# hank-kuo-cs/Volumetric-Primitives-Net

Hardware: NVIDIA B200
Metric: primitive-loss fwd+bwd samples/sec (higher is better)
Workload: dtype f32

## Files before the change

### volumetric-primitives-net_b200/csrc/chamfer_prep.cu

```cuda
#include "common.cuh"

namespace vpn {

constexpr int kSortThreads = 1024;
constexpr int kSortMaxM = 16384;
constexpr int kBlk = 128;

__device__ __forceinline__ float prep_inf() { return __int_as_float(0x7f800000); }
__device__ __forceinline__ unsigned spread6(unsigned x) {
  x = (x | (x << 8)) & 0x0000300Fu;
  x = (x | (x << 4)) & 0x000030C3u;
  x = (x | (x << 2)) & 0x00009249u;
  return x;
}
__device__ __forceinline__ u64 prep_pk(float a, float b) { u64 r; asm("mov.b64 %0, {%1,%2};" : "=l"(r) : "f"(a), "f"(b)); return r; }
__device__ __forceinline__ void prep_upk(u64 v, float& a, float& b) { asm("mov.b64 {%0,%1}, %2;" : "=f"(a), "=f"(b) : "l"(v)); }
__device__ __forceinline__ u64 prep_sub2(u64 a, u64 b) { u64 r; asm("sub.rn.f32x2 %0, %1, %2;" : "=l"(r) : "l"(a), "l"(b)); return r; }
__device__ __forceinline__ u64 prep_mul2(u64 a, u64 b) { u64 r; asm("mul.rn.f32x2 %0, %1, %2;" : "=l"(r) : "l"(a), "l"(b)); return r; }
__device__ __forceinline__ u64 prep_fma2(u64 a, u64 b, u64 c) { u64 r; asm("fma.rn.f32x2 %0, %1, %2, %3;" : "=l"(r) : "l"(a), "l"(b), "l"(c)); return r; }

__device__ __forceinline__ float warp_min_f(float v) { float r; asm volatile("redux.sync.min.f32 %0, %1, 0xffffffff;" : "=f"(r) : "f"(v)); return r; }
__device__ __forceinline__ float warp_max_f(float v) { float r; asm volatile("redux.sync.max.f32 %0, %1, 0xffffffff;" : "=f"(r) : "f"(v)); return r; }

__device__ __forceinline__ void prep_block_box(float (&lo)[3], float (&hi)[3], unsigned amu, float (*red)[7]) {
// ... 318 lines not shown
    __syncthreads();
    pp.mark();
    return;
  }
  const int b = blockIdx.x;
  const float* T = p2 + (size_t)b * M * 3;
  float* Ts = p2s + (size_t)b * M * 3;
  float4* Tv = p2v + (size_t)b * nchunks * kBlk;
  int* pm = perm + (size_t)b * M;
  float* cb = cbox + (size_t)b * nchunks * 8;
  if (M <= 8 * kSortThreads) prep_sort_targets<8>(T, Ts, Tv, pm, cb, tmax + b, M, sort_targets, deterministic, nchunks, cnt, start, ent, wsum, red, pp);
  else prep_sort_targets<16>(T, Ts, Tv, pm, cb, tmax + b, M, sort_targets, deterministic, nchunks, cnt, start, ent, wsum, red, pp);
}

constexpr int kNearRows = 8, kRepsRows = 4;
constexpr int kNearCols = 32, kRepsCols = 4;
constexpr int kMaxNear = 32, kMaxReps = 128;
constexpr int kGapCap = 1024;
constexpr int kBoundWarps = 4;

__device__ __forceinline__ float box_gap2(const float* __restrict__ a, const float* __restrict__ b) {
  float s = 0.f;
#pragma unroll
  for (int k = 0; k < 3; ++k) {
    const float g = fmaxf(0.f, fmaxf(a[k] - b[3 + k], b[k] - a[3 + k]));
    s = fmaf(g, g, s);
  }
  return s;
}

__global__ void __launch_bounds__(kBoundWarps * 32, 8)
chamfer_prune_bounds_kernel(const float* __restrict__ p1, const float* __restrict__ p2s,
                            const float* __restrict__ rbox, const float* __restrict__ cbox,
                            float* __restrict__ rthr, float* __restrict__ cub, int P, int M, int nrb, int nchunks,
                            int near_rows, int reps_rows, int near_cols, int reps_cols, int gap_cap) {
  extern __shared__ unsigned s_gap[];
  __shared__ float4 s_reps[kBoundWarps][2 * kMaxReps];
  __shared__ int s_sel[kBoundWarps][kMaxNear];
  const int b = blockIdx.y, lane = threadIdx.x & 31, warp = threadIdx.x >> 5;
  const int id = blockIdx.x * kBoundWarps + warp;
  if (id >= nrb + nchunks) return;
  unsigned* gap = s_gap + warp * gap_cap; float4* reps = s_reps[warp]; int* sel = s_sel[warp];
  const bool is_row = id >= nchunks;
  const int blk = is_row ? id - nchunks : id;
  const int n_mine = is_row ? P : M, n_other = is_row ? M : P;
  const float* mine = (is_row ? p1 + (size_t)b * P * 3 : p2s + (size_t)b * M * 3);
  const float* other = (is_row ? p2s + (size_t)b * M * 3 : p1 + (size_t)b * P * 3);
  const int nob = is_row ? nchunks : nrb;
  const float* obox = (is_row ? cbox + (size_t)b * nchunks * 8 : rbox + (size_t)b * nrb * 8);
  const int near = is_row ? near_rows : near_cols, per = is_row ? reps_rows : reps_cols;
  const float* mb = is_row ? rbox + ((size_t)b * nrb + blk) * 8 : cbox + ((size_t)b * nchunks + blk) * 8;
  float mybox[6];
#pragma unroll
  for (int k = 0; k < 6; ++k) mybox[k] = mb[k];
  float x[4], y[4], z[4]; bool valid[4];
#pragma unroll
  for (int u = 0; u < 4; ++u) {
    const int idx = blk * kBlk + u * 32 + lane;
    valid[u] = idx < n_mine;
    x[u] = y[u] = z[u] = 0.f;
    if (valid[u]) { x[u] = mine[3 * (size_t)idx]; y[u] = mine[3 * (size_t)idx + 1]; z[u] = mine[3 * (size_t)idx + 2]; }
  }
  const int stride = (nob + kGapCap - 1) / kGapCap, ncand = (nob + stride - 1) / stride;
  unsigned lmin = 0xffffffffu;
  for (int c = lane; c < ncand; c += 32) {
    const float4* ob = reinterpret_cast<const float4*>(obox + (size_t)c * stride * 8);
    const float4 o0 = ob[0], o1 = ob[1];
    const float other_box[6] = {o0.x, o0.y, o0.z, o0.w, o1.x, o1.y};
    const float g = box_gap2(mybox, other_box);
    const unsigned k = ((g == g) ? (__float_as_uint(g) & ~0x3ffu) : 0x7f800000u) | (unsigned)c;
    gap[c] = k;
    lmin = min(lmin, k);
  }
  const int nsel = min(near, ncand);
  for (int s = 0; s < nsel; ++s) {
    const unsigned w = __reduce_min_sync(0xffffffffu, lmin);
    const int bi = (w == 0xffffffffu) ? -1 : (int)(w & 0x3ffu);
    if (lane == 0) sel[s] = bi < 0 ? 0 : bi;
    if (bi >= 0 && (bi & 31) == lane) {
      gap[bi] = 0xffffffffu;
      lmin = 0xffffffffu;
      for (int c = lane; c < ncand; c += 32) lmin = min(lmin, gap[c]);
    }
  }
  __syncwarp();
  const int nrep = nsel * per;
  for (int i = lane; i < nrep; i += 32) {
    const int ob = sel[i / per] * stride;
    int o = ob * kBlk + (i % per) * (kBlk / per);
    o = min(o, n_other - 1);
    const float qx = other[3 * (size_t)o], qy = other[3 * (size_t)o + 1], qz = other[3 * (size_t)o + 2];
    reps[2 * i] = make_float4(qx, qx, qy, qy); reps[2 * i + 1] = make_float4(qz, qz, 0.f, 0.f);
  }
  __syncwarp();
  const u64 x01 = prep_pk(x[0], x[1]), x23 = prep_pk(x[2], x[3]), y01 = prep_pk(y[0], y[1]), y23 = prep_pk(y[2], y[3]),
            z01 = prep_pk(z[0], z[1]), z23 = prep_pk(z[2], z[3]);
  float ub[4] = {prep_inf(), prep_inf(), prep_inf(), prep_inf()};
  for (int r = 0; r < nrep; ++r) {
    const ulonglong2 qa = *reinterpret_cast<const ulonglong2*>(&reps[2 * r]);
    const u64 qz = *reinterpret_cast<const u64*>(&reps[2 * r + 1]);
    const u64 dx0 = prep_sub2(x01, qa.x), dy0 = prep_sub2(y01, qa.y), dz0 = prep_sub2(z01, qz);
    const u64 dx1 = prep_sub2(x23, qa.x), dy1 = prep_sub2(y23, qa.y), dz1 = prep_sub2(z23, qz);
    const u64 s0 = prep_fma2(dz0, dz0, prep_fma2(dy0, dy0, prep_mul2(dx0, dx0)));
    const u64 s1 = prep_fma2(dz1, dz1, prep_fma2(dy1, dy1, prep_mul2(dx1, dx1)));
    float a, c, e, f;
    prep_upk(s0, a, c); prep_upk(s1, e, f);
    ub[0] = fminf(ub[0], a); ub[1] = fminf(ub[1], c); ub[2] = fminf(ub[2], e); ub[3] = fminf(ub[3], f);
  }
  float m = 0.f;
#pragma unroll
  for (int u = 0; u < 4; ++u) if (valid[u]) m = fmaxf(m, ub[u]);
  m = warp_max_f(m);
  if (lane == 0) { if (is_row) rthr[(size_t)b * nrb + blk] = m; else cub[(size_t)b * nchunks + blk] = m; }
}

int chamfer_row_segment() { return kRowSeg; }

size_t chamfer_sort_smem_bytes(int M) {
  if (M > kSortMaxM) return 0;
  return (size_t)kCells * 8 + (((size_t)M * 4 + 15) & ~(size_t)15);
}

int chamfer_prep_launch(const float* p1, const float* p2, float* p2s, float4* p2v, int* perm, float* cbox, float* rbox, float* rthr,
                        float* cub, float* tmax, float* p1s, int* rperm, unsigned long long* stats, int B, int P, int M, cudaStream_t s) {
  const int nchunks = (M + kBlk - 1) / kBlk, nrb = (P + kBlk - 1) / kBlk;
  const size_t smem_t = chamfer_sort_smem_bytes(M);
  const size_t smem_r = (size_t)kCells * 8 + (size_t)kRowSeg * 4 + (size_t)kRowSeg * 12;
  const size_t smem = smem_t > smem_r ? smem_t : smem_r;
  static DeviceOnce once;
  if (set_dyn_smem(chamfer_sort_targets_kernel, kCells * 8 + kSortMaxM * 4 + kRowSeg * 12, once) != cudaSuccess) {
    vpn_set_error("chamfer prep: smem attribute"); return VPN_ERR_CUDA;
  }
  const long long seg_ctas = (long long)((P + kRowSeg - 1) / kRowSeg) * B;
  if (B + seg_ctas > 0x7fffffffLL) { vpn_set_error("chamfer prep: too many row segments"); return VPN_ERR_SHAPE; }
  chamfer_sort_targets_kernel<<<(unsigned)(B + seg_ctas), kSortThreads, smem, s>>>(p2, p2s, p2v, perm, cbox, tmax, M, smem_t > 0 ? 1 : 0, nchunks,
                                                                                   p1, p1s, rperm, rbox, P, nrb, B,
                                                                                   tuning_value(kTunePrepDeterministic) == 1 ? 1 : 0,
                                                                                   tuning_value(kTunePrepProbe) == 1 ? stats : nullptr);
  int rc = vpn_check_launch("chamfer_sort_targets_kernel");
  if (rc) return rc;
  auto pick = [](int key, int dflt, int cap) { const int v = tuning_value(key); return (v >= 1 && v <= cap && (key == kTunePrepNearRows || key == kTunePrepNearCols || v == 1 || v == 2 || v == 4)) ? v : dflt; };
  const int most = nrb > nchunks ? nrb : nchunks;
  const int gap_cap = most >= kGapCap ? kGapCap : ((most + 31) & ~31);
  chamfer_prune_bounds_kernel<<<dim3((nrb + nchunks + kBoundWarps - 1) / kBoundWarps, B), kBoundWarps * 32,
                                (size_t)kBoundWarps * gap_cap * sizeof(unsigned), s>>>(
      p1s, p2s, rbox, cbox, rthr, cub, P, M, nrb, nchunks, pick(kTunePrepNearRows, kNearRows, kMaxNear), pick(kTunePrepRepsRows, kRepsRows, 4),
      pick(kTunePrepNearCols, kNearCols, kMaxNear), pick(kTunePrepRepsCols, kRepsCols, 4), gap_cap);
  return vpn_check_launch("chamfer_prune_bounds_kernel");
}

}
```

### volumetric-primitives-net_b200/csrc/chamfer_tc.cu

```cuda
#include <cuda_fp16.h>
#include "common.cuh"

namespace vpn {

constexpr int kTcBlk = 128;
constexpr int kTcEpiWarps = 16;
constexpr int kTcThreads = (kTcEpiWarps + 4) * 32;
constexpr int kTcBlkBytes = kTcBlk * 32;
constexpr float kTcBig = 1.0e30f;
constexpr int kTcDefaultHunits = 0;

__device__ __forceinline__ uint32_t tc_smem_u32(const void* p) { return (uint32_t)__cvta_generic_to_shared(p); }
__device__ __forceinline__ float tc_inf() { return __int_as_float(0x7f800000); }

__device__ __forceinline__ uint64_t tc_desc(uint32_t saddr) {
  return (uint64_t)((saddr & 0x3FFFF) >> 4) | ((uint64_t)(128 >> 4) << 16) | ((uint64_t)(256 >> 4) << 32) | (1ull << 46);
}
constexpr uint32_t kTcIdesc = (1u << 4) | (0u << 7) | (0u << 10) | ((uint32_t)(2 * kTcBlk >> 3) << 17) | ((uint32_t)(kTcBlk >> 4) << 24);

constexpr uint32_t kTcIdescHalf = (1u << 4) | (0u << 7) | (0u << 10) | ((uint32_t)(kTcBlk >> 3) << 17) | ((uint32_t)(kTcBlk >> 4) << 24);
constexpr uint32_t kTcIdescHalfF16 = (0u << 4) | (0u << 7) | (0u << 10) | ((uint32_t)(kTcBlk >> 3) << 17) | ((uint32_t)(kTcBlk >> 4) << 24);

__device__ __forceinline__ void tc_mma(uint32_t d_tmem, uint64_t a, uint64_t b, uint32_t accumulate, uint32_t idesc = kTcIdesc) {
#if defined(VPN_TC_VARIANT) && VPN_TC_VARIANT == 3
// ... 181 lines not shown
  uint32_t u23 = tc_min_s16x2(__byte_perm(m2, m3, 0x5410), __byte_perm(m2, m3, 0x7632));
  u01 = tc_max_s16x2(u01, 0u); u23 = tc_max_s16x2(u23, 0u);
  const float2 f01 = __half22float2(*reinterpret_cast<const __half2*>(&u01)), f23 = __half22float2(*reinterpret_cast<const __half2*>(&u23));
  u[0] = f01.x; u[1] = f01.y; u[2] = f23.x; u[3] = f23.y;
  return fminf(tc_min3(u[0], u[1], u[2]), u[3]);
}

__device__ __forceinline__ u64 tc_spread_nibbles(uint32_t v) {
  u64 x = v;
  x = (x | (x << 16)) & 0x0000FFFF0000FFFFull;
  x = (x | (x << 8)) & 0x00FF00FF00FF00FFull;
  x = (x | (x << 4)) & 0x0F0F0F0F0F0F0F0Full;
  return x;
}
__device__ __forceinline__ float tc_box_gap2(const float* __restrict__ a, const float* __restrict__ b) {
  float s = 0.f;
#pragma unroll
  for (int k = 0; k < 3; ++k) {
    const float g = fmaxf(0.f, fmaxf(a[k] - b[3 + k], b[k] - a[3 + k]));
    s = fmaf(g, g, s);
  }
  return s;
}

__device__ __forceinline__ bool tc_pass_needed(int j, int nc, int NB, const uint32_t* raw) {
  const uint32_t live = ~raw[2 * j] | ((2 * j + 1 < nc) ? ~raw[2 * j + 1] : 0u);
  return (live & ((1u << NB) - 1u)) != 0u;
}

constexpr int kPlanThreads = 128;
static_assert(kPlanThreads == kTcPlanWords, "one plan word per thread");
__global__ void __launch_bounds__(kPlanThreads)
chamfer_tc_plan_kernel(const float* __restrict__ cbox, const float* __restrict__ rbox, const float* __restrict__ rthr,
                       const float* __restrict__ cub, uint32_t* __restrict__ plan_masks, int* __restrict__ plan_work,
                       int ncta, int ntiles, int nsplit, int nrb_total, int NB, int nchunks, int cps) {
  __shared__ uint32_t skipR[64], skipC[64];
  __shared__ int s_live[kPlanThreads / 32];
  __shared__ float4 s_rbox[16][2];
  __shared__ float s_rthr[16];
  const int tid = threadIdx.x, lane = tid & 31, warp = tid >> 5;
  const int cta = blockIdx.x;
  const int tile_i = cta % ntiles, split = (cta / ntiles) % nsplit, b = cta / (ntiles * nsplit);
  const int c_first = split * cps, nc = min(nchunks, c_first + cps) - c_first;
  if (tid < 64) { skipR[tid] = 0u; skipC[tid] = 0u; }
  if (tid < 2 * NB) {
    const int r = tid >> 1, rb = tile_i * NB + r;
    if (rb < nrb_total) s_rbox[r][tid & 1] = reinterpret_cast<const float4*>(rbox + ((size_t)b * nrb_total + rb) * 8)[tid & 1];
  } else if (tid >= 32 && tid < 32 + NB) {
    const int r = tid - 32, rb = tile_i * NB + r;
    s_rthr[r] = (rb < nrb_total) ? __fmul_ru(rthr[(size_t)b * nrb_total + rb], 1.00001f) : 0.f;
  }
  __syncthreads();
  {
    const int c = tid & 63, r0 = (tid >> 6) * (NB / 2);
    if (c < nc) {
      const float4 c0 = reinterpret_cast<const float4*>(cbox + ((size_t)b * nchunks + c_first + c) * 8)[0];
      const float4 c1 = reinterpret_cast<const float4*>(cbox + ((size_t)b * nchunks + c_first + c) * 8)[1];
      const float cb8[8] = {c0.x, c0.y, c0.z, c0.w, c1.x, c1.y, c1.z, c1.w};
      const float ub = __fmul_ru(cub[(size_t)b * nchunks + c_first + c], 1.00001f);
      uint32_t mr = 0u, mc = 0u;
      for (int r = r0; r < r0 + NB / 2; ++r) {
        bool pr = true, pc = true;
        if (tile_i * NB + r < nrb_total) {
          const float4 a0 = s_rbox[r][0], a1 = s_rbox[r][1];
          const float rb8[8] = {a0.x, a0.y, a0.z, a0.w, a1.x, a1.y, a1.z, a1.w};
          const float gap2 = tc_box_gap2(rb8, cb8);
          pr = gap2 > s_rthr[r];
          pc = gap2 > ub;
        }
        mr |= pr ? (1u << r) : 0u;
        mc |= pc ? (1u << r) : 0u;
      }
      atomicOr(&skipR[c], mr);
      atomicOr(&skipC[c], mc);
    }
  }
  __syncthreads();
  uint32_t* out = plan_masks + (size_t)cta * kTcPlanWords;
  int live = 0;
  {
    const int c = tid & 63;
    const uint32_t m = (c < nc) ? (tid < 64 ? skipR[c] : skipC[c]) : 0xffffffffu;
    if (c < nc) live = NB - __popc(m & ((1u << NB) - 1u));
    out[tid] = m;
  }
#pragma unroll
  for (int o = 16; o > 0; o >>= 1) live += __shfl_xor_sync(0xffffffffu, live, o);
  if (lane == 0) s_live[warp] = live;
  __syncthreads();
  if (tid == 0) plan_work[cta] = s_live[0] + s_live[1] + s_live[2] + s_live[3];
}

constexpr int kOrderThreads = 1024, kOrderBins = 2112;
__global__ void __launch_bounds__(kOrderThreads)
chamfer_tc_order_kernel(const int* __restrict__ plan_work, int* __restrict__ plan_order, int ncta) {
  __shared__ int hist[kOrderBins];
  const int tid = threadIdx.x;
  for (int i = tid; i < kOrderBins; i += kOrderThreads) hist[i] = 0;
  __syncthreads();
  for (int i = tid; i < ncta; i += kOrderThreads) atomicAdd(&hist[min(max(plan_work[i], 0), kOrderBins - 1)], 1);
  __syncthreads();
  {
    constexpr int kPer = (kOrderBins + kOrderThreads - 1) / kOrderThreads;
    __shared__ int wsum[32];
    const int lane = tid & 31, warp = tid >> 5;
    int cnt[kPer], sum = 0;
#pragma unroll
    for (int k = 0; k < kPer; ++k) { const int w = kOrderBins - 1 - (tid * kPer + k); cnt[k] = (w >= 0) ? hist[w] : 0; sum += cnt[k]; }
    int inc = sum;
#pragma unroll
    for (int o = 1; o < 32; o <<= 1) { const int t = __shfl_up_sync(0xffffffffu, inc, o); if (lane >= o) inc += t; }
    if (lane == 31) wsum[warp] = inc;
    __syncthreads();
    if (warp == 0) {
      const int w = wsum[lane];
// ... 363 lines not shown
          else if (v < bv || j == 0) { bv = v; bj = j; }
        }
      }
      mn[i] = bv; ix[i] = bj;
    }
  }
}

__global__ void __launch_bounds__(256)
chamfer_tc_bounds_kernel(const float* __restrict__ p2, float* __restrict__ tmax, int M) {
  __shared__ float red[8];
  const float* T = p2 + (size_t)blockIdx.x * M * 3;
  float m = 0.f;
  for (int i = threadIdx.x; i < 3 * M; i += 256) {
    const float v = fabsf(T[i]);
    m = (v <= m) ? m : v;
  }
#pragma unroll
  for (int o = 16; o > 0; o >>= 1) { const float x = __shfl_xor_sync(0xffffffffu, m, o); m = (x <= m) ? m : x; }
  if ((threadIdx.x & 31) == 0) red[threadIdx.x >> 5] = m;
  __syncthreads();
  if (threadIdx.x == 0) {
    for (int w = 1; w < 8; ++w) m = (red[w] <= m) ? m : red[w];
    tmax[blockIdx.x] = m;
  }
}

size_t chamfer_tc_smem_bytes(int NB) { return tc_smem_bytes(NB); }
int chamfer_tc_plan_words() { return kTcPlanWords; }


int chamfer_tc_launch(const float* p1, const float* p2, float* rbest, u64* rmask, float* cbest, u64* cmask,
                      float2* tslack, int* fallback, float* tmax, const float* cbox, const float* rbox, const float* rthr,
                      const float* cub, u64* stats, uint32_t* plan_masks, int* plan_work, int* plan_order, int with_bounds,
                      int B, int P, int M, int NB, int ntiles, int nsplit, int nchunks, int cps, cudaStream_t s) {
  static DeviceOnce once;
  const size_t smem = tc_smem_bytes(NB);
  {
    cudaError_t e = set_dyn_smem(chamfer_tc_kernel<0>, (int)tc_smem_bytes(16), once);
    for (int k = 0; k < 4 && e == cudaSuccess; ++k) {
      void (*kern)(const float*, const float*, float*, u64*, float*, u64*, float2*, int*, const float*, const uint32_t*, const int*, u64*,
                   int, int, int, int, int, int, int) = k == 0 ? chamfer_tc_kernel<1> : (k == 1 ? chamfer_tc_kernel<2> : (k == 2 ? chamfer_tc_kernel<3> : chamfer_tc_kernel<4>));
      static DeviceOnce more[4];
      e = set_dyn_smem(kern, (int)tc_smem_bytes(16), more[k]);
    }
    if (e != cudaSuccess) { vpn_set_error("chamfer tc: smem attribute: %s", cudaGetErrorString(e)); return VPN_ERR_CUDA; }
  }
  int rc;
  if (with_bounds) {
    chamfer_tc_bounds_kernel<<<B, 256, 0, s>>>(p2, tmax, M);
    if ((rc = vpn_check_launch("chamfer_tc_bounds_kernel"))) return rc;
  }
  const long long ncta_ll = (long long)ntiles * nsplit * B;
  if (ncta_ll > 0x7fffffffLL) { vpn_set_error("chamfer tc: too many tiles"); return VPN_ERR_SHAPE; }
  const int ncta = (int)ncta_ll;
  if (cbox != nullptr) {
    chamfer_tc_plan_kernel<<<ncta, kPlanThreads, 0, s>>>(
        cbox, rbox, rthr, cub, plan_masks, plan_work, ncta, ntiles, nsplit, (P + kTcBlk - 1) / kTcBlk, NB, nchunks, cps);
    if ((rc = vpn_check_launch("chamfer_tc_plan_kernel"))) return rc;
    chamfer_tc_order_kernel<<<1, kOrderThreads, 0, s>>>(plan_work, plan_order, ncta);
    if ((rc = vpn_check_launch("chamfer_tc_order_kernel"))) return rc;
  }
  const int tune_h = tuning_value(kTuneTcHunits);
  const int hunits = (tune_h >= 1 && tune_h <= 5) ? tune_h - 1 : kTcDefaultHunits;
#define VPN_TC_LAUNCH(H) chamfer_tc_kernel<H><<<ncta, kTcThreads, smem, s>>>(p1, p2, rbest, rmask, cbest, cmask, tslack, fallback, tmax, \
                                                   cbox ? plan_masks : nullptr, cbox ? plan_order : nullptr, stats, \
                                                   ntiles, nsplit, P, M, NB, nchunks, cps)
  switch (hunits) {
    case 0: VPN_TC_LAUNCH(0); break;
    case 1: VPN_TC_LAUNCH(1); break;
    case 2: VPN_TC_LAUNCH(2); break;
    case 3: VPN_TC_LAUNCH(3); break;
    default: VPN_TC_LAUNCH(4); break;
  }
#undef VPN_TC_LAUNCH
  return vpn_check_launch("chamfer_tc_kernel");
}

int chamfer_flagged_launch(const float* p1, const float* p2, float* min1, int* idx1, float* min2, int* idx2,
                           const int* fallback, int B, int P, int M, cudaStream_t s) {
  chamfer_flagged_kernel<<<dim3(32, B), 256, 0, s>>>(p1, p2, min1, idx1, min2, idx2, fallback, P, M);
  return vpn_check_launch("chamfer_flagged_kernel");
}

}
```

### volumetric-primitives-net_b200/csrc/chamfer_tiled.cu

```cuda
#include <cstdlib>
#include <mutex>
#include <type_traits>
#include "common.cuh"

namespace vpn {

enum { MODE_EXACT = 0, MODE_DIFF = 1, MODE_EXPAND = 2, MODE_TC = 3 };

constexpr int kTThreads = 256;
constexpr int kTWarps = kTThreads / 32;
constexpr int kCW = 128;
constexpr int kMaxChunksPerSplit = 64;
constexpr float kBig = 1.0e30f;

__device__ __forceinline__ u64 pk(float a, float b) { u64 r; asm("mov.b64 %0, {%1,%2};" : "=l"(r) : "f"(a), "f"(b)); return r; }
__device__ __forceinline__ void upk(u64 v, float& a, float& b) { asm("mov.b64 {%0,%1}, %2;" : "=f"(a), "=f"(b) : "l"(v)); }
__device__ __forceinline__ u64 add2(u64 a, u64 b) { u64 r; asm("add.rn.f32x2 %0, %1, %2;" : "=l"(r) : "l"(a), "l"(b)); return r; }
__device__ __forceinline__ u64 sub2(u64 a, u64 b) { u64 r; asm("sub.rn.f32x2 %0, %1, %2;" : "=l"(r) : "l"(a), "l"(b)); return r; }
__device__ __forceinline__ u64 mul2(u64 a, u64 b) { u64 r; asm("mul.rn.f32x2 %0, %1, %2;" : "=l"(r) : "l"(a), "l"(b)); return r; }
__device__ __forceinline__ u64 fma2(u64 a, u64 b, u64 c) { u64 r; asm("fma.rn.f32x2 %0, %1, %2, %3;" : "=l"(r) : "l"(a), "l"(b), "l"(c)); return r; }
__device__ __forceinline__ float min3f(float a, float b, float c) { float r; asm("min.f32 %0, %1, %2, %3;" : "=f"(r) : "f"(a), "f"(b), "f"(c)); return r; }
__device__ __forceinline__ float warp_min_f32(float a) { float r; asm volatile("redux.sync.min.f32 %0, %1, 0xffffffff;" : "=f"(r) : "f"(a)); return r; }
__device__ __forceinline__ float inf_f() { return __int_as_float(0x7f800000); }

// ... 559 lines not shown
          }
          int at;
          const int st = unit_scan(d, dm, lane, &at);
          u64 kv = ~0ull;
          if (st == 1) kv = ((u64)__float_as_uint(sqrtf(dm)) << 32) | (unsigned)__float_as_int(rows[base_row + at].w);
          else if (st == 2) kv = unit_exact_walk(tx, ty, tz, rows + base_row, 0, 1);
          best = kv < best ? kv : best;
        }
        if (best != ~0ull) atomicMin(&key2[(size_t)b * M + col], best);
      }
      __syncthreads();
    }
  }
}

__global__ void chamfer_unpack_key_kernel(const u64* __restrict__ key, float* __restrict__ mn, int* __restrict__ idx, size_t n,
                                          const int* __restrict__ skip, int per_sample, const int* __restrict__ perm) {
  size_t i = (size_t)blockIdx.x * blockDim.x + threadIdx.x;
  if (i >= n) return;
  const size_t smp = i / (size_t)per_sample;
  if (skip && skip[smp]) return;
  u64 k = key[i];
  const size_t o = perm ? smp * (size_t)per_sample + (size_t)perm[i] : i;
  mn[o] = __uint_as_float((unsigned)(k >> 32));
  idx[o] = (int)(unsigned)(k & 0xffffffffu);
}

struct TiledPlan { int R, ntiles, nchunks, nsplit, cps, tc, TM; };

size_t chamfer_tc_smem_bytes(int NB);
int chamfer_tc_plan_words();
int chamfer_tc_launch(const float* p1, const float* p2, float* rbest, u64* rmask, float* cbest, u64* cmask,
                      float2* tslack, int* fallback, float* tmax, const float* cbox, const float* rbox, const float* rthr,
                      const float* cub, u64* stats, unsigned* plan_masks, int* plan_work, int* plan_order, int with_bounds,
                      int B, int P, int M, int NB, int ntiles, int nsplit, int nchunks, int cps, cudaStream_t s);
int chamfer_prep_launch(const float* p1, const float* p2, float* p2s, float4* p2v, int* perm, float* cbox, float* rbox, float* rthr,
                        float* cub, float* tmax, float* p1s, int* rperm, unsigned long long* stats, int B, int P, int M, cudaStream_t s);
int chamfer_flagged_launch(const float* p1, const float* p2, float* min1, int* idx1, float* min2, int* idx2,
                           const int* fallback, int B, int P, int M, cudaStream_t s);

static void finish_plan(TiledPlan& pl, int B, long long slots, int min_cps) {
  long long base = (long long)pl.ntiles * B;
  long long s = (4 * slots + base - 1) / base;
  long long smin = (pl.nchunks + kMaxChunksPerSplit - 1) / kMaxChunksPerSplit;
  long long smax = pl.nchunks / min_cps;
  if (s > smax) s = smax;
  if (s < smin) s = smin;
  if (s > pl.nchunks) s = pl.nchunks;
  if (s < 1) s = 1;
  pl.cps = (int)((pl.nchunks + s - 1) / s);
  pl.nsplit = (pl.nchunks + pl.cps - 1) / pl.cps;
}

static bool make_plan(int B, int P, int M, int sm_count, TiledPlan& pl) {
  if (P < 1024 || M < kCW || B < 1) return false;
  pl.tc = 0;
  pl.nchunks = (M + kCW - 1) / kCW;
  const int rs[3] = {16, 8, 4};
  int pick = 4;
  for (int k = 0; k < 3; ++k) {
    int R = rs[k], tm = kTThreads * R;
    long long nt = (P + tm - 1) / tm;
    double waste = (double)(nt * tm) / P;
    long long slots = (long long)sm_count * (R <= 8 ? 2 : 1);
    if (waste <= 1.26 && nt * B * pl.nchunks >= 2 * slots) { pick = R; break; }
  }
  { int r = tuning_value(kTuneTiledR); if (r == 4 || r == 8 || r == 16) pick = r; }
  pl.R = pick;
  pl.TM = kTThreads * pl.R;
  pl.ntiles = (P + pl.TM - 1) / pl.TM;
  finish_plan(pl, B, (long long)sm_count * (pl.R <= 8 ? 2 : 1), 1);
  return pl.nsplit <= 65535;
}

static bool make_plan_tc(int B, int P, int M, int sm_count, TiledPlan& pl) {
  if (P < 512 || M < kCW || B < 1) return false;
  pl.tc = 1;
  pl.nchunks = (M + kCW - 1) / kCW;
  const int nbs[3] = {16, 8, 4};
  int pick = 4;
  for (int k = 0; k < 3; ++k) {
    int nb = nbs[k], tm = 128 * nb;
    long long nt = (P + tm - 1) / tm;
    double waste = (double)(nt * tm) / P;
    if (waste <= 1.26 && nt * B * pl.nchunks >= 2LL * sm_count * 8) { pick = nb; break; }
  }
  { int r = tuning_value(kTuneTcNb); if (r == 4 || r == 8 || r == 16) pick = r; }
  pl.R = pick;
  pl.TM = 128 * pl.R;
  pl.ntiles = (P + pl.TM - 1) / pl.TM;
  finish_plan(pl, B, sm_count, 4);
  return pl.nsplit <= 65535;
}

static size_t al256(size_t x) { return (x + 255) & ~(size_t)255; }

struct TiledWs { size_t rbest, rmask, cbest, cmask, tslack, fallback, tmax, cthr, key2, p2s, p2v, perm, cbox, rbox, rthr, cub, pmask, pwork, porder, p1s, rperm, total; };
static TiledWs ws_layout(int B, int P, int M, const TiledPlan& pl) {
  TiledWs w; size_t o = 0;
  w.rbest = o; o += al256((size_t)B * pl.nsplit * P * 4);
  w.rmask = o; o += al256((size_t)B * pl.nsplit * P * 8 * (pl.tc ? 4 : 1));
  w.cbest = o; o += al256((size_t)B * pl.ntiles * M * 4);
  w.cmask = o; o += al256((size_t)B * pl.ntiles * M * (pl.tc ? 8 : 4));
  w.tslack = o; o += al256((size_t)B * pl.ntiles * 8);
  w.fallback = o; o += al256((size_t)B * 4 + 8 + 128);
  w.tmax = o; o += al256((size_t)B * 4);
  w.cthr = o; o += al256((size_t)B * M * 4);
  w.key2 = o; o += al256((size_t)B * M * 8);
  w.p2s = w.p2v = w.perm = w.cbox = w.rbox = w.rthr = w.cub = w.pmask = w.pwork = w.porder = w.p1s = w.rperm = 0;
  if (pl.tc) {
    const size_t nrb = (size_t)(P + 127) / 128;
    w.p2s = o; o += al256((size_t)B * M * 12);
    w.p2v = o; o += al256((size_t)B * pl.nchunks * kCW * 16);
    w.perm = o; o += al256((size_t)B * M * 4);
    w.cbox = o; o += al256((size_t)B * pl.nchunks * 32);
    w.rbox = o; o += al256((size_t)B * nrb * 32);
    w.rthr = o; o += al256((size_t)B * nrb * 4);
    w.cub = o; o += al256((size_t)B * pl.nchunks * 4);
    const size_t ncta = (size_t)pl.ntiles * pl.nsplit * B;
    w.pmask = o; o += al256(ncta * (size_t)chamfer_tc_plan_words() * 4);
    w.pwork = o; o += al256(ncta * 4);
    w.porder = o; o += al256(ncta * 4);
    w.p1s = o; o += al256((size_t)B * P * 12);
    w.rperm = o; o += al256((size_t)B * P * 4);
  }
  w.total = o;
  return w;
}

static bool plan_for(int mode, int B, int P, int M, TiledPlan& pl) {
  const int kPlanSms = device_sm_count();
  if (mode == MODE_TC) return make_plan_tc(B, P, M, kPlanSms, pl);
  if (mode >= 0) return make_plan(B, P, M, kPlanSms, pl);
  return make_plan_tc(B, P, M, kPlanSms, pl) || make_plan(B, P, M, kPlanSms, pl);
}

int chamfer_tiled_supported(int B, int P, int M, int mode) {
  TiledPlan pl;
  return plan_for(mode, B, P, M, pl) ? 1 : 0;
}

int chamfer_tiled_uses_tc(int B, int P, int M, int mode) {
  TiledPlan pl;
  return (plan_for(mode, B, P, M, pl) && pl.tc) ? 1 : 0;
}

size_t chamfer_tiled_workspace_bytes(int B, int P, int M, int mode) {
  TiledPlan pl;
  if (!plan_for(mode, B, P, M, pl)) return 0;
  return ws_layout(B, P, M, pl).total;
}
// ... 81 lines not shown
        cudaEventCreateWithFlags(&ss.fork, cudaEventDisableTiming) != cudaSuccess ||
        cudaEventCreateWithFlags(&ss.join, cudaEventDisableTiming) != cudaSuccess) { cudaGetLastError(); return nullptr; }
    ss.ok = true;
  }
  return &ss;
}

int chamfer_tiled_fwd(const float* p1, const float* p2, float* min1, int* idx1, float* min2, int* idx2,
                      int B, int P, int M, void* ws_, size_t ws_bytes, int mode, cudaStream_t s, cudaEvent_t* ev) {
  TiledPlan pl;
  if (!plan_for(mode, B, P, M, pl)) { vpn_set_error("chamfer tiled: unsupported shape"); return VPN_ERR_SHAPE; }
  if (mode < 0) mode = pl.tc ? MODE_TC : MODE_EXPAND;
  TiledWs wl = ws_layout(B, P, M, pl);
  if (ws_bytes < wl.total) { vpn_set_error("chamfer tiled: workspace too small (%zu < %zu)", ws_bytes, wl.total); return VPN_ERR_WORKSPACE; }
  char* ws = reinterpret_cast<char*>(ws_);
  int* fallback = reinterpret_cast<int*>(ws + wl.fallback);
  const int* skip = nullptr;
  int rc;
  if (ev) cudaEventRecord(ev[0], s);
  const size_t flag_bytes = (((size_t)B * 4 + 7) & ~(size_t)7) + 128;
  if (mode == MODE_EXPAND || mode == MODE_TC) {
    if (cudaMemsetAsync(fallback, 0, flag_bytes, s) != cudaSuccess) { vpn_set_error("chamfer tiled: memset failed"); return VPN_ERR_CUDA; }
  }
  const float* p2w = p2;
  const int* perm = nullptr;
  const float4* p2v = nullptr;
  const float* p1w = p1;
  const int* rperm = nullptr;
  if (mode == MODE_TC) {
    float* p2s = reinterpret_cast<float*>(ws + wl.p2s);
    int* pm = reinterpret_cast<int*>(ws + wl.perm);
    float* cbox = reinterpret_cast<float*>(ws + wl.cbox); float* rbox = reinterpret_cast<float*>(ws + wl.rbox);
    float* rthr = reinterpret_cast<float*>(ws + wl.rthr); float* cub = reinterpret_cast<float*>(ws + wl.cub);
    float* tmax = reinterpret_cast<float*>(ws + wl.tmax);
    u64* stats = reinterpret_cast<u64*>(ws + wl.fallback + (((size_t)B * 4 + 7) & ~(size_t)7));
    const bool prune = tuning_value(kTuneTcPrune) != 2;
    if (prune) {
      float4* pv = reinterpret_cast<float4*>(ws + wl.p2v);
      float* p1s = reinterpret_cast<float*>(ws + wl.p1s);
      int* rp = reinterpret_cast<int*>(ws + wl.rperm);
      if ((rc = chamfer_prep_launch(p1, p2, p2s, pv, pm, cbox, rbox, rthr, cub, tmax, p1s, rp, stats, B, P, M, s))) return rc;
      p2w = p2s; perm = pm; p2v = pv; p1w = p1s; rperm = rp;
    }
    rc = chamfer_tc_launch(p1w, p2w, reinterpret_cast<float*>(ws + wl.rbest), reinterpret_cast<u64*>(ws + wl.rmask),
                           reinterpret_cast<float*>(ws + wl.cbest), reinterpret_cast<u64*>(ws + wl.cmask),
                           reinterpret_cast<float2*>(ws + wl.tslack), fallback, tmax, prune ? cbox : nullptr, rbox, rthr, cub, stats,
                           reinterpret_cast<unsigned*>(ws + wl.pmask), reinterpret_cast<int*>(ws + wl.pwork),
                           reinterpret_cast<int*>(ws + wl.porder), prune ? 0 : 1, B, P, M, pl.R, pl.ntiles, pl.nsplit, pl.nchunks,
                           pl.cps, s);
    if (rc) return rc;
    if (ev) cudaEventRecord(ev[1], s);
    if ((rc = chamfer_flagged_launch(p1, p2, min1, idx1, min2, idx2, fallback, B, P, M, s))) return rc;
    skip = fallback;
  } else {
    if ((rc = launch_any(mode, p1, p2, ws, wl, pl, B, P, M, 0, s))) return rc;
    if (ev) cudaEventRecord(ev[1], s);
    if (mode == MODE_EXPAND) {
      if ((rc = launch_any(MODE_DIFF, p1, p2, ws, wl, pl, B, P, M, 1, s))) return rc;
    }
  }
  if (ev) cudaEventRecord(ev[2], s);
  SideStream* side = tuning_value(kTuneSerialRecovery) ? nullptr : side_stream_for(s);
  std::unique_lock<std::mutex> side_lock;
  cudaStream_t sc = s;
  if (side) {
    side_lock = std::unique_lock<std::mutex>(side->mu);
    if (cudaEventRecord(side->fork, s) == cudaSuccess && cudaStreamWaitEvent(side->s, side->fork, 0) == cudaSuccess) sc = side->s;
    else { cudaGetLastError(); side = nullptr; side_lock.unlock(); }
  }
  {
    static DeviceOnce once_rows;
    const size_t smem_rows = kRowsFixedSmem + (size_t)(pl.nchunks < kSegChunks ? pl.nchunks : kSegChunks) * kCW * sizeof(float4);
    if (set_dyn_smem(chamfer_recover_rows_kernel, (int)(kRowsFixedSmem + kSegChunks * kCW * sizeof(float4)), once_rows) != cudaSuccess) {
      vpn_set_error("chamfer tiled: smem attribute (rows recovery)"); return VPN_ERR_CUDA;
    }
    const int nblk = (P + kRowGroup - 1) / kRowGroup;
    const long long nitems = (long long)nblk * B;
    if (nitems > 0x7fffffffLL) { vpn_set_error("chamfer tiled: too many row blocks"); return VPN_ERR_SHAPE; }
    const int sms = device_sm_count();
// ... 45 lines not shown
```

Measured before the change: 34490.

## Refine chamfer tile pruning with per-warp sub-block bounding boxes

The bounds kernel now also emits, for each 128-point block, four 32-point sub-boxes and a per-sub-block upper bound. The plan kernel re-tests every surviving row/column block pair at 32-point granularity and marks the pair skippable when no sub-box pair can beat its bound. This aims to prune more tensor-core tiles in the chamfer nearest-neighbour search. The cost is extra warp reductions and stores in prep, more shared memory and a second pass with atomics in the plan kernel, and more workspace.

```diff
diff --git a/volumetric-primitives-net_b200/csrc/chamfer_prep.cu b/volumetric-primitives-net_b200/csrc/chamfer_prep.cu
--- a/volumetric-primitives-net_b200/csrc/chamfer_prep.cu
+++ b/volumetric-primitives-net_b200/csrc/chamfer_prep.cu
@@ -374,8 +374,9 @@
 __global__ void __launch_bounds__(kBoundWarps * 32, 8)
 chamfer_prune_bounds_kernel(const float* __restrict__ p1, const float* __restrict__ p2s,
                             const float* __restrict__ rbox, const float* __restrict__ cbox,
-                            float* __restrict__ rthr, float* __restrict__ cub, int P, int M, int nrb, int nchunks,
-                            int near_rows, int reps_rows, int near_cols, int reps_cols, int gap_cap) {
+                            float* __restrict__ rthr, float* __restrict__ cub, float* __restrict__ rbox_u,
+                            float* __restrict__ cbox_u, float* __restrict__ rthr_u, float* __restrict__ cub_u, int P, int M, int nrb,
+                            int nchunks, int near_rows, int reps_rows, int near_cols, int reps_cols, int gap_cap) {
   extern __shared__ unsigned s_gap[];
   __shared__ float4 s_reps[kBoundWarps][2 * kMaxReps];
   __shared__ int s_sel[kBoundWarps][kMaxNear];
@@ -403,6 +404,22 @@
     x[u] = y[u] = z[u] = 0.f;
     if (valid[u]) { x[u] = mine[3 * (size_t)idx]; y[u] = mine[3 * (size_t)idx + 1]; z[u] = mine[3 * (size_t)idx + 2]; }
   }
+  const size_t ublk = is_row ? (size_t)b * nrb + blk : (size_t)b * nchunks + blk;
+  float* ubnd = (is_row ? rthr_u : cub_u) + ublk * 4;
+  {
+    float* ubox = (is_row ? rbox_u : cbox_u) + ublk * 32;
+#pragma unroll
+    for (int u = 0; u < 4; ++u) {
+      const float l0 = warp_min_f(valid[u] ? x[u] : prep_inf()), l1 = warp_min_f(valid[u] ? y[u] : prep_inf()),
+                  l2 = warp_min_f(valid[u] ? z[u] : prep_inf());
+      const float h0 = warp_max_f(valid[u] ? x[u] : -prep_inf()), h1 = warp_max_f(valid[u] ? y[u] : -prep_inf()),
+                  h2 = warp_max_f(valid[u] ? z[u] : -prep_inf());
+      if (lane == 0) {
+        reinterpret_cast<float4*>(ubox + u * 8)[0] = make_float4(l0, l1, l2, h0);
+        reinterpret_cast<float4*>(ubox + u * 8)[1] = make_float4(h1, h2, 0.f, 0.f);
+      }
+    }
+  }
   const int stride = (nob + kGapCap - 1) / kGapCap, ncand = (nob + stride - 1) / stride;
   unsigned lmin = 0xffffffffu;
   for (int c = lane; c < ncand; c += 32) {
@@ -451,8 +468,11 @@
   }
   float m = 0.f;
 #pragma unroll
-  for (int u = 0; u < 4; ++u) if (valid[u]) m = fmaxf(m, ub[u]);
-  m = warp_max_f(m);
+  for (int u = 0; u < 4; ++u) {
+    const float mu = warp_max_f(valid[u] ? ub[u] : 0.f);
+    m = fmaxf(m, mu);
+    if (lane == 0) ubnd[u] = mu;
+  }
   if (lane == 0) { if (is_row) rthr[(size_t)b * nrb + blk] = m; else cub[(size_t)b * nchunks + blk] = m; }
 }
 
@@ -464,7 +484,8 @@
 }
 
 int chamfer_prep_launch(const float* p1, const float* p2, float* p2s, float4* p2v, int* perm, float* cbox, float* rbox, float* rthr,
-                        float* cub, float* tmax, float* p1s, int* rperm, unsigned long long* stats, int B, int P, int M, cudaStream_t s) {
+                        float* cub, float* rbox_u, float* cbox_u, float* rthr_u, float* cub_u, float* tmax, float* p1s, int* rperm,
+                        unsigned long long* stats, int B, int P, int M, cudaStream_t s) {
   const int nchunks = (M + kBlk - 1) / kBlk, nrb = (P + kBlk - 1) / kBlk;
   const size_t smem_t = chamfer_sort_smem_bytes(M);
   const size_t smem_r = (size_t)kCells * 8 + (size_t)kRowSeg * 4 + (size_t)kRowSeg * 12;
@@ -486,7 +507,7 @@
   const int gap_cap = most >= kGapCap ? kGapCap : ((most + 31) & ~31);
   chamfer_prune_bounds_kernel<<<dim3((nrb + nchunks + kBoundWarps - 1) / kBoundWarps, B), kBoundWarps * 32,
                                 (size_t)kBoundWarps * gap_cap * sizeof(unsigned), s>>>(
-      p1s, p2s, rbox, cbox, rthr, cub, P, M, nrb, nchunks, pick(kTunePrepNearRows, kNearRows, kMaxNear), pick(kTunePrepRepsRows, kRepsRows, 4),
+      p1s, p2s, rbox, cbox, rthr, cub, rbox_u, cbox_u, rthr_u, cub_u, P, M, nrb, nchunks, pick(kTunePrepNearRows, kNearRows, kMaxNear), pick(kTunePrepRepsRows, kRepsRows, 4),
       pick(kTunePrepNearCols, kNearCols, kMaxNear), pick(kTunePrepRepsCols, kRepsCols, 4), gap_cap);
   return vpn_check_launch("chamfer_prune_bounds_kernel");
 }
diff --git a/volumetric-primitives-net_b200/csrc/chamfer_tc.cu b/volumetric-primitives-net_b200/csrc/chamfer_tc.cu
--- a/volumetric-primitives-net_b200/csrc/chamfer_tc.cu
+++ b/volumetric-primitives-net_b200/csrc/chamfer_tc.cu
@@ -237,17 +237,27 @@
 static_assert(kPlanThreads == kTcPlanWords, "one plan word per thread");
 __global__ void __launch_bounds__(kPlanThreads)
 chamfer_tc_plan_kernel(const float* __restrict__ cbox, const float* __restrict__ rbox, const float* __restrict__ rthr,
-                       const float* __restrict__ cub, uint32_t* __restrict__ plan_masks, int* __restrict__ plan_work,
-                       int ncta, int ntiles, int nsplit, int nrb_total, int NB, int nchunks, int cps) {
+                       const float* __restrict__ cub, const float* __restrict__ cbox_u, const float* __restrict__ rbox_u,
+                       const float* __restrict__ cub_u, const float* __restrict__ rthr_u, uint32_t* __restrict__ plan_masks,
+                       int* __restrict__ plan_work, int ncta, int ntiles, int nsplit, int nrb_total, int NB, int nchunks, int cps,
+                       int P, int M) {
   __shared__ uint32_t skipR[64], skipC[64];
   __shared__ int s_live[kPlanThreads / 32];
   __shared__ float4 s_rbox[16][2];
   __shared__ float s_rthr[16];
+  __shared__ float4 s_rubox[16][4][2];
+  __shared__ float s_rub[16][4];
+  __shared__ float4 s_cubox[64][4][2];
+  __shared__ float s_cub[64][4];
+  __shared__ uint16_t s_item[64 * 16];
+  __shared__ int s_nitem;
+  __shared__ uint32_t liveR[64], liveC[64];
   const int tid = threadIdx.x, lane = tid & 31, warp = tid >> 5;
   const int cta = blockIdx.x;
   const int tile_i = cta % ntiles, split = (cta / ntiles) % nsplit, b = cta / (ntiles * nsplit);
   const int c_first = split * cps, nc = min(nchunks, c_first + cps) - c_first;
-  if (tid < 64) { skipR[tid] = 0u; skipC[tid] = 0u; }
+  if (tid < 64) { skipR[tid] = 0u; skipC[tid] = 0u; liveR[tid] = 0u; liveC[tid] = 0u; }
+  if (tid == 0) s_nitem = 0;
   if (tid < 2 * NB) {
     const int r = tid >> 1, rb = tile_i * NB + r;
     if (rb < nrb_total) s_rbox[r][tid & 1] = reinterpret_cast<const float4*>(rbox + ((size_t)b * nrb_total + rb) * 8)[tid & 1];
@@ -255,14 +265,27 @@
     const int r = tid - 32, rb = tile_i * NB + r;
     s_rthr[r] = (rb < nrb_total) ? __fmul_ru(rthr[(size_t)b * nrb_total + rb], 1.00001f) : 0.f;
   }
+  for (int i = tid; i < 8 * NB; i += kPlanThreads) {
+    const int r = i >> 3, rb = tile_i * NB + r;
+    if (rb < nrb_total) s_rubox[r][(i >> 1) & 3][i & 1] = reinterpret_cast<const float4*>(rbox_u + ((size_t)b * nrb_total + rb) * 32)[i & 7];
+  }
+  if (tid < 4 * NB) {
+    const int r = tid >> 2, rb = tile_i * NB + r;
+    s_rub[r][tid & 3] = (rb < nrb_total) ? __fmul_ru(rthr_u[((size_t)b * nrb_total + rb) * 4 + (tid & 3)], 1.00001f) : 0.f;
+  }
+  for (int i = tid; i < 8 * nc; i += kPlanThreads)
+    s_cubox[i >> 3][(i >> 1) & 3][i & 1] = reinterpret_cast<const float4*>(cbox_u + ((size_t)b * nchunks + c_first) * 32)[i];
+  for (int i = tid; i < 4 * nc; i += kPlanThreads)
+    s_cub[i >> 2][i & 3] = __fmul_ru(cub_u[((size_t)b * nchunks + c_first) * 4 + i], 1.00001f);
   __syncthreads();
   {
     const int c = tid & 63, r0 = (tid >> 6) * (NB / 2);
     if (c < nc) {
-      const float4 c0 = reinterpret_cast<const float4*>(cbox + ((size_t)b * nchunks + c_first + c) * 8)[0];
-      const float4 c1 = reinterpret_cast<const float4*>(cbox + ((size_t)b * nchunks + c_first + c) * 8)[1];
+      const size_t cg = (size_t)b * nchunks + c_first + c;
+      const float4 c0 = reinterpret_cast<const float4*>(cbox + cg * 8)[0];
+      const float4 c1 = reinterpret_cast<const float4*>(cbox + cg * 8)[1];
       const float cb8[8] = {c0.x, c0.y, c0.z, c0.w, c1.x, c1.y, c1.z, c1.w};
-      const float ub = __fmul_ru(cub[(size_t)b * nchunks + c_first + c], 1.00001f);
+      const float ub = __fmul_ru(cub[cg], 1.00001f);
       uint32_t mr = 0u, mc = 0u;
       for (int r = r0; r < r0 + NB / 2; ++r) {
         bool pr = true, pc = true;
@@ -272,6 +295,7 @@
           const float gap2 = tc_box_gap2(rb8, cb8);
           pr = gap2 > s_rthr[r];
           pc = gap2 > ub;
+          if (!(pr && pc)) s_item[atomicAdd(&s_nitem, 1)] = (uint16_t)(c << 4 | r);
         }
         mr |= pr ? (1u << r) : 0u;
         mc |= pc ? (1u << r) : 0u;
@@ -279,13 +303,36 @@
       atomicOr(&skipR[c], mr);
       atomicOr(&skipC[c], mc);
     }
+  }
+  __syncthreads();
+  for (int i = tid; i < 4 * s_nitem; i += kPlanThreads) {
+    const int item = s_item[i >> 2], qr = i & 3, c = item >> 4, r = item & 15;
+    if ((tile_i * NB + r) * kTcBlk + qr * 32 >= P) continue;
+    const int ccols = M - (c_first + c) * kTcBlk;
+    const int ncu = ccols >= kTcBlk ? 4 : (ccols + 31) >> 5;
+    const float4 q0 = s_rubox[r][qr][0], q1 = s_rubox[r][qr][1];
+    const float ru8[8] = {q0.x, q0.y, q0.z, q0.w, q1.x, q1.y, q1.z, q1.w};
+    const float rbound = s_rub[r][qr];
+    bool lr = false, lc = false;
+#pragma unroll
+    for (int uc = 0; uc < 4; ++uc) {
+      if (uc >= ncu) break;
+      const float4 u0 = s_cubox[c][uc][0], u1 = s_cubox[c][uc][1];
+      const float cu8[8] = {u0.x, u0.y, u0.z, u0.w, u1.x, u1.y, u1.z, u1.w};
+      const float g2 = tc_box_gap2(ru8, cu8);
+      lr = lr || !(g2 > rbound);
+      lc = lc || !(g2 > s_cub[c][uc]);
+    }
+    if (lr) atomicOr(&liveR[c], 1u << r);
+    if (lc) atomicOr(&liveC[c], 1u << r);
   }
   __syncthreads();
   uint32_t* out = plan_masks + (size_t)cta * kTcPlanWords;
   int live = 0;
   {
     const int c = tid & 63;
-    const uint32_t m = (c < nc) ? (tid < 64 ? skipR[c] : skipC[c]) : 0xffffffffu;
+    const uint32_t nbmask = (1u << NB) - 1u;
+    const uint32_t m = (c < nc) ? (tid < 64 ? skipR[c] | (~liveR[c] & nbmask) : skipC[c] | (~liveC[c] & nbmask)) : 0xffffffffu;
     if (c < nc) live = NB - __popc(m & ((1u << NB) - 1u));
     out[tid] = m;
   }
@@ -715,7 +762,8 @@
 
 int chamfer_tc_launch(const float* p1, const float* p2, float* rbest, u64* rmask, float* cbest, u64* cmask,
                       float2* tslack, int* fallback, float* tmax, const float* cbox, const float* rbox, const float* rthr,
-                      const float* cub, u64* stats, uint32_t* plan_masks, int* plan_work, int* plan_order, int with_bounds,
+                      const float* cub, const float* rbox_u, const float* cbox_u, const float* rthr_u, const float* cub_u,
+                      u64* stats, uint32_t* plan_masks, int* plan_work, int* plan_order, int with_bounds,
                       int B, int P, int M, int NB, int ntiles, int nsplit, int nchunks, int cps, cudaStream_t s) {
   static DeviceOnce once;
   const size_t smem = tc_smem_bytes(NB);
@@ -739,7 +787,8 @@
   const int ncta = (int)ncta_ll;
   if (cbox != nullptr) {
     chamfer_tc_plan_kernel<<<ncta, kPlanThreads, 0, s>>>(
-        cbox, rbox, rthr, cub, plan_masks, plan_work, ncta, ntiles, nsplit, (P + kTcBlk - 1) / kTcBlk, NB, nchunks, cps);
+        cbox, rbox, rthr, cub, cbox_u, rbox_u, cub_u, rthr_u, plan_masks, plan_work, ncta, ntiles, nsplit,
+        (P + kTcBlk - 1) / kTcBlk, NB, nchunks, cps, P, M);
     if ((rc = vpn_check_launch("chamfer_tc_plan_kernel"))) return rc;
     chamfer_tc_order_kernel<<<1, kOrderThreads, 0, s>>>(plan_work, plan_order, ncta);
     if ((rc = vpn_check_launch("chamfer_tc_order_kernel"))) return rc;
diff --git a/volumetric-primitives-net_b200/csrc/chamfer_tiled.cu b/volumetric-primitives-net_b200/csrc/chamfer_tiled.cu
--- a/volumetric-primitives-net_b200/csrc/chamfer_tiled.cu
+++ b/volumetric-primitives-net_b200/csrc/chamfer_tiled.cu
@@ -615,10 +615,12 @@
 int chamfer_tc_plan_words();
 int chamfer_tc_launch(const float* p1, const float* p2, float* rbest, u64* rmask, float* cbest, u64* cmask,
                       float2* tslack, int* fallback, float* tmax, const float* cbox, const float* rbox, const float* rthr,
-                      const float* cub, u64* stats, unsigned* plan_masks, int* plan_work, int* plan_order, int with_bounds,
+                      const float* cub, const float* rbox_u, const float* cbox_u, const float* rthr_u, const float* cub_u,
+                      u64* stats, unsigned* plan_masks, int* plan_work, int* plan_order, int with_bounds,
                       int B, int P, int M, int NB, int ntiles, int nsplit, int nchunks, int cps, cudaStream_t s);
 int chamfer_prep_launch(const float* p1, const float* p2, float* p2s, float4* p2v, int* perm, float* cbox, float* rbox, float* rthr,
-                        float* cub, float* tmax, float* p1s, int* rperm, unsigned long long* stats, int B, int P, int M, cudaStream_t s);
+                        float* cub, float* rbox_u, float* cbox_u, float* rthr_u, float* cub_u, float* tmax, float* p1s, int* rperm,
+                        unsigned long long* stats, int B, int P, int M, cudaStream_t s);
 int chamfer_flagged_launch(const float* p1, const float* p2, float* min1, int* idx1, float* min2, int* idx2,
                            const int* fallback, int B, int P, int M, cudaStream_t s);
 
@@ -678,7 +680,8 @@
 
 static size_t al256(size_t x) { return (x + 255) & ~(size_t)255; }
 
-struct TiledWs { size_t rbest, rmask, cbest, cmask, tslack, fallback, tmax, cthr, key2, p2s, p2v, perm, cbox, rbox, rthr, cub, pmask, pwork, porder, p1s, rperm, total; };
+struct TiledWs { size_t rbest, rmask, cbest, cmask, tslack, fallback, tmax, cthr, key2, p2s, p2v, perm, cbox, rbox, rthr, cub, rbox_u, cbox_u, rthr_u, cub_u, pmask, pwork, porder, p1s,
+                 rperm, total; };
 static TiledWs ws_layout(int B, int P, int M, const TiledPlan& pl) {
   TiledWs w; size_t o = 0;
   w.rbest = o; o += al256((size_t)B * pl.nsplit * P * 4);
@@ -690,7 +693,8 @@
   w.tmax = o; o += al256((size_t)B * 4);
   w.cthr = o; o += al256((size_t)B * M * 4);
   w.key2 = o; o += al256((size_t)B * M * 8);
-  w.p2s = w.p2v = w.perm = w.cbox = w.rbox = w.rthr = w.cub = w.pmask = w.pwork = w.porder = w.p1s = w.rperm = 0;
+  w.p2s = w.p2v = w.perm = w.cbox = w.rbox = w.rthr = w.cub = w.rbox_u = w.cbox_u = w.rthr_u = w.cub_u = 0;
+  w.pmask = w.pwork = w.porder = w.p1s = w.rperm = 0;
   if (pl.tc) {
     const size_t nrb = (size_t)(P + 127) / 128;
     w.p2s = o; o += al256((size_t)B * M * 12);
@@ -700,6 +704,10 @@
     w.rbox = o; o += al256((size_t)B * nrb * 32);
     w.rthr = o; o += al256((size_t)B * nrb * 4);
     w.cub = o; o += al256((size_t)B * pl.nchunks * 4);
+    w.rbox_u = o; o += al256((size_t)B * nrb * 4 * 32);
+    w.cbox_u = o; o += al256((size_t)B * pl.nchunks * 4 * 32);
+    w.rthr_u = o; o += al256((size_t)B * nrb * 4 * 4);
+    w.cub_u = o; o += al256((size_t)B * pl.nchunks * 4 * 4);
     const size_t ncta = (size_t)pl.ntiles * pl.nsplit * B;
     w.pmask = o; o += al256(ncta * (size_t)chamfer_tc_plan_words() * 4);
     w.pwork = o; o += al256(ncta * 4);
@@ -847,6 +855,8 @@
     int* pm = reinterpret_cast<int*>(ws + wl.perm);
     float* cbox = reinterpret_cast<float*>(ws + wl.cbox); float* rbox = reinterpret_cast<float*>(ws + wl.rbox);
     float* rthr = reinterpret_cast<float*>(ws + wl.rthr); float* cub = reinterpret_cast<float*>(ws + wl.cub);
+    float* rbox_u = reinterpret_cast<float*>(ws + wl.rbox_u); float* cbox_u = reinterpret_cast<float*>(ws + wl.cbox_u);
+    float* rthr_u = reinterpret_cast<float*>(ws + wl.rthr_u); float* cub_u = reinterpret_cast<float*>(ws + wl.cub_u);
     float* tmax = reinterpret_cast<float*>(ws + wl.tmax);
     u64* stats = reinterpret_cast<u64*>(ws + wl.fallback + (((size_t)B * 4 + 7) & ~(size_t)7));
     const bool prune = tuning_value(kTuneTcPrune) != 2;
@@ -854,12 +864,14 @@
       float4* pv = reinterpret_cast<float4*>(ws + wl.p2v);
       float* p1s = reinterpret_cast<float*>(ws + wl.p1s);
       int* rp = reinterpret_cast<int*>(ws + wl.rperm);
-      if ((rc = chamfer_prep_launch(p1, p2, p2s, pv, pm, cbox, rbox, rthr, cub, tmax, p1s, rp, stats, B, P, M, s))) return rc;
+      if ((rc = chamfer_prep_launch(p1, p2, p2s, pv, pm, cbox, rbox, rthr, cub, rbox_u, cbox_u, rthr_u, cub_u, tmax, p1s, rp, stats, B,
+                                   P, M, s))) return rc;
       p2w = p2s; perm = pm; p2v = pv; p1w = p1s; rperm = rp;
     }
     rc = chamfer_tc_launch(p1w, p2w, reinterpret_cast<float*>(ws + wl.rbest), reinterpret_cast<u64*>(ws + wl.rmask),
                            reinterpret_cast<float*>(ws + wl.cbest), reinterpret_cast<u64*>(ws + wl.cmask),
-                           reinterpret_cast<float2*>(ws + wl.tslack), fallback, tmax, prune ? cbox : nullptr, rbox, rthr, cub, stats,
+                           reinterpret_cast<float2*>(ws + wl.tslack), fallback, tmax, prune ? cbox : nullptr, rbox, rthr, cub, rbox_u,
+                           cbox_u, rthr_u, cub_u, stats,
                            reinterpret_cast<unsigned*>(ws + wl.pmask), reinterpret_cast<int*>(ws + wl.pwork),
                            reinterpret_cast<int*>(ws + wl.porder), prune ? 0 : 1, B, P, M, pl.R, pl.ntiles, pl.nsplit, pl.nchunks,
                            pl.cps, s);
```

Measured after the change: 35690 (median of 6 runs). +3.5%, better.
